# study-game-engines/directx-renderer-kurth

Measured on AMD Instinct MI355X. Metric: physics steps/sec at 100k rigid bodies, higher is better.
Workload: dtype f32; 1 GPU; c3: 100k mixed colliders (sphere/capsule/OBB), dt 1/120 s, 30 solver iterations; bodies=100000, broadphase_pairs=611032, manifolds=251275, contacts=317267, joints=0, recoveries=0, parallelism=1 gpu

## Files before the change

### directx-renderer-kurth_amd/csrc/k_broad.hip

```cpp
#include "world.h"
#include <rocprim/rocprim.hpp>

#define CELL_BIAS (1 << 20)
#define CELL_MASK ((1u << 21) - 1u)
#define EMPTY_CELL 0xFFFFFFFFu

MI_DEV u64 packCell(i32 ix, i32 iy, i32 iz) { return ((u64)(u32)(ix & CELL_MASK)) | ((u64)(u32)(iy & CELL_MASK) << 21) | ((u64)(u32)(iz & CELL_MASK) << 42); }
MI_DEV u32 hashCell(u64 k, u32 mask)
{
	k ^= k >> 30; k *= 0xbf58476d1ce4e5b9ull; k ^= k >> 27; k *= 0x94d049bb133111ebull; k ^= k >> 31;
	return (u32)k & mask;
}
MI_DEV i32 cellCoord(float v, float invCell)
{
	float c = floorf(v * invCell);
	c = fminf(fmaxf(c, -(float)(CELL_BIAS - 2)), (float)(CELL_BIAS - 2));
	return (i32)c + CELL_BIAS;
}
MI_DEV u32 cellTag(i32 ix, i32 iy, i32 iz) { return ((u32)ix & 0x3FFu) | (((u32)iy & 0x3FFu) << 10) | (((u32)iz & 0x3FFu) << 20); }
MI_DEV bool aabbOverlap(float4 amin, float4 amax, float4 bmin, float4 bmax)
{
	if (amax.x < bmin.x || amin.x > bmax.x) return false;
	if (amax.y < bmin.y || amin.y > bmax.y) return false;
	if (amax.z < bmin.z || amin.z > bmax.z) return false;
	return true;
}

__global__ void __launch_bounds__(256) k_cell_assign(const u32* __restrict__ activeCols, u32 hashMask, const float4* __restrict__ aabbMin, const float4* __restrict__ aabbMax,
	u32* __restrict__ counters, u32* __restrict__ hashKey, u32* __restrict__ cellCount)
{
	const u32 gid = blockIdx.x * blockDim.x + threadIdx.x;
	if (gid == 0) { counters[CTR_FIRST_LARGE] = 0xFFFFFFFFu; counters[CTR_FIRST_INACTIVE] = 0xFFFFFFFFu; counters[CTR_PAIR_OVERFLOW] = 0u; }
	const u32 n = counters[CTR_ACTIVE_COLS];
	float maxExtent = fmaxf(__uint_as_float(counters[CTR_CELL_SIZE]), 1e-3f);
	float cell = maxExtent * 1.001f;
	float invCell = 1.f / cell;
	for (u32 a = gid; a < n; a += gridDim.x * blockDim.x)
	{
		const u32 i = activeCols[a];
		float4 mn = aabbMin[i], mx = aabbMax[i];
		float e = fmaxf(fmaxf(mx.x - mn.x, mx.y - mn.y), mx.z - mn.z);
		u32 h;
		if (mn.x > mx.x) { h = hashMask + 2; }
		else if (e > maxExtent) { h = hashMask + 1; }
		else { h = hashCell(packCell(cellCoord(mn.x, invCell), cellCoord(mn.y, invCell), cellCoord(mn.z, invCell)), hashMask); }
		hashKey[i] = h;
		atomicAdd(&cellCount[h], 1u);
	}
}

__global__ void __launch_bounds__(256) k_cell_place(const u32* __restrict__ counters, const u32* __restrict__ activeCols, const u32* __restrict__ hashKey, u32* __restrict__ cellBase, u32* __restrict__ tmpIdx)
{
	const u32 n = counters[CTR_ACTIVE_COLS];
	for (u32 a = blockIdx.x * blockDim.x + threadIdx.x; a < n; a += gridDim.x * blockDim.x) { const u32 i = activeCols[a]; tmpIdx[atomicAdd(&cellBase[hashKey[i]], 1u)] = i; }
}
__global__ void __launch_bounds__(256) k_cell_rank(u32* __restrict__ counters, u32 hashMask, const u32* __restrict__ hashKey, const u32* __restrict__ cellBase, const u32* __restrict__ cellCount, const u32* __restrict__ tmpIdx,
	const float4* __restrict__ aabbMin, const float4* __restrict__ aabbMax, float4* __restrict__ sBox, u32* __restrict__ cellRange)
{
	const u32 n = counters[CTR_ACTIVE_COLS];
	const float cell = fmaxf(__uint_as_float(counters[CTR_CELL_SIZE]), 1e-3f) * 1.001f;
	const float invCell = 1.f / cell;
	if (blockIdx.x == 0 && threadIdx.x == 0) counters[CTR_CELL_SIZE_USED] = counters[CTR_CELL_SIZE];
	for (u32 t = blockIdx.x * blockDim.x + threadIdx.x; t < n; t += gridDim.x * blockDim.x)
	{
		const u32 i = tmpIdx[t], h = hashKey[i], end = cellBase[h], start = end - cellCount[h];
		u32 rank = t - start;
		if (h != hashMask + 2u) { rank = 0; for (u32 u = start; u < end; ++u) rank += tmpIdx[u] < i ? 1u : 0u; }
		const u32 pos = start + rank;
		float4 mn = aabbMin[i], mx = aabbMax[i];
		mx.w = __uint_as_float(cellTag(cellCoord(mn.x, invCell), cellCoord(mn.y, invCell), cellCoord(mn.z, invCell)));
		mn.w = __uint_as_float(i);
		sBox[2 * pos] = mn; sBox[2 * pos + 1] = mx;
		if (t == start)
		{
			if (h <= hashMask) { cellRange[2 * h] = start; cellRange[2 * h + 1] = end; }
			else counters[h == hashMask + 1 ? CTR_FIRST_LARGE : CTR_FIRST_INACTIVE] = start;
		}
	}
}

#define PAIR_SLAB 32
#define PAIR_LANES 16
#define PAIR_NO_TAG 0xFFFFFFFFu
enum { MODE_SLAB = 0, MODE_WRITE = 1 };
MI_DEV uint2 pairRange(const uint4* ranges, u32 r) { return make_uint2(ranges[r].x, ranges[r].y); }
MI_DEV const float4* pairBox(const float4* __restrict__ sBox, u32 u) { return (const float4*)((const char*)sBox + u * 32u); }
template <int MODE>
__global__ void __launch_bounds__(256) k_pairs(u32 nc, u32 hashMask, const float4* __restrict__ sBox, const uint2* __restrict__ cellRange, u32* __restrict__ counters,
	u32* __restrict__ pairCount, const u32* __restrict__ pairOffset, uint2* __restrict__ out, u32 pairCap)
{
	__shared__ uint4 sRange[256 / PAIR_LANES][PAIR_LANES];
	u32 gid = blockIdx.x * blockDim.x + threadIdx.x;
	u32 t = gid / PAIR_LANES, g = gid % PAIR_LANES;
	const uint4* __restrict__ ranges = sRange[threadIdx.x / PAIR_LANES];
	bool valid = t < nc;
	u32 nEnd = min(counters[CTR_FIRST_INACTIVE], min(nc, counters[CTR_ACTIVE_COLS]));
	u32 firstLarge = min(counters[CTR_FIRST_LARGE], nEnd);
	bool live = valid && t < nEnd;
	if (MODE == MODE_WRITE) live = live && pairCount[t] > PAIR_SLAB;
	float4 amin = make_float4(0.f, 0.f, 0.f, 0.f), amax = amin;
	u32 me = 0;
	u32 s = 0, len = 0, ntag = PAIR_NO_TAG;
	if (live)
	{
		amin = sBox[2 * t]; amax = sBox[2 * t + 1];
		me = __float_as_uint(amin.w);
		if (t >= firstLarge) { if (g == 0) { s = firstLarge; len = t - firstLarge; } }
		else if (g == 14) { s = firstLarge; len = nEnd - firstLarge; }
		else if (g < 14)
		{
			const float invCell = 1.f / (fmaxf(__uint_as_float(counters[CTR_CELL_SIZE_USED]), 1e-3f) * 1.001f);
			i32 ix = cellCoord(amin.x, invCell), iy = cellCoord(amin.y, invCell), iz = cellCoord(amin.z, invCell);
			i32 o = 13 + (i32)g;
			i32 dz = o / 9 - 1, dy = (o / 3) % 3 - 1, dx = o % 3 - 1;
			bool reach = true;
			if (dx > 0 && cellCoord(amax.x, invCell) == ix) reach = false;
			if (dy > 0 && cellCoord(amax.y, invCell) == iy) reach = false;
			if (dz > 0 && cellCoord(amax.z, invCell) == iz) reach = false;
			if (reach)
			{
				ntag = cellTag(ix + dx, iy + dy, iz + dz);
				u32 h = hashCell(packCell(ix + dx, iy + dy, iz + dz), hashMask);
				uint2 range = cellRange[h];
				if (range.x != EMPTY_CELL) { s = range.x; const u32 e = g == 0 ? min(range.y, t) : range.y; len = e > s ? e - s : 0u; }
			}
		}
	}
	u32 end = len;
	for (u32 d = 1; d < PAIR_LANES; d <<= 1) { u32 v = __shfl_up(end, d, PAIR_LANES); if (g >= d) end += v; }
	sRange[threadIdx.x / PAIR_LANES][g] = make_uint4(end, s - (end - len), ntag, 0u);
	__syncthreads();
	const u32 T = ranges[PAIR_LANES - 1].x;
	const u32 chunk = (T + PAIR_LANES - 1u) / PAIR_LANES;
	const u32 lo = min(g * chunk, T), hi = min(lo + chunk, T);
	u32 r0 = 0;
#pragma unroll
	for (u32 k = 0; k < PAIR_LANES - 1u; ++k) r0 += ranges[k].x <= lo ? 1u : 0u;
	u32 n = 0;
	u32 hit0 = 0, hit1 = 0, hit2 = 0, hit3 = 0;
	if (lo < hi)
	{
		u32 r = r0; uint2 cur = pairRange(ranges, r);
		for (u32 p = lo; p < hi; p += 4u)
		{
			float4 bmin[4], bmax[4]; u32 from = 0;
#pragma unroll
			for (u32 k = 0; k < 4u; ++k) if (p + k < hi)
			{
				while (p + k >= cur.x) cur = pairRange(ranges, ++r);
				const float4* box = pairBox(sBox, cur.y + p + k);
				from |= r << (4u * k); bmin[k] = box[0]; bmax[k] = box[1];
			}
#pragma unroll
			for (u32 k = 0; k < 4u; ++k)
			{
				if (p + k >= hi) continue;
				const u32 want = ranges[(from >> (4u * k)) & 15u].z;
				if (want != PAIR_NO_TAG && __float_as_uint(bmax[k].w) != want) continue;
				if (aabbOverlap(amin, amax, bmin[k], bmax[k]))
				{
					u32 partner = __float_as_uint(bmin[k].w);
					if (n == 0) hit0 = partner; else if (n == 1) hit1 = partner; else if (n == 2) hit2 = partner; else if (n == 3) hit3 = partner;
					++n;
				}
			}
		}
	}
	u32 incl = n;
	for (u32 d = 1; d < PAIR_LANES; d <<= 1) { u32 v = __shfl_up(incl, d, PAIR_LANES); if (g >= d) incl += v; }
	u32 total = __shfl(incl, PAIR_LANES - 1, PAIR_LANES);
	u32 pos = incl - n;
	if (MODE == MODE_SLAB && valid && g == 0) { pairCount[t] = live ? total : 0; if (total > PAIR_SLAB) counters[CTR_PAIR_OVERFLOW] = 1; }
	if (!n) return;
	size_t base = (MODE == MODE_WRITE) ? (size_t)pairOffset[t] : (size_t)t * PAIR_SLAB;
	u32 room = (MODE == MODE_WRITE) ? 0xFFFFFFFFu : PAIR_SLAB;
	if (n <= 4)
	{
		for (u32 k = 0; k < n; ++k)
		{
			u32 partner = k == 0 ? hit0 : (k == 1 ? hit1 : (k == 2 ? hit2 : hit3));
			if (pos + k < room && (MODE == MODE_SLAB || base + pos + k < pairCap)) out[base + pos + k] = make_uint2(me, partner);
		}
		return;
	}
	u32 r = r0; uint2 cur = pairRange(ranges, r);
	for (u32 p = lo; p < hi; ++p)
	{
		while (p >= cur.x) cur = pairRange(ranges, ++r);
		const float4* box = pairBox(sBox, cur.y + p);
		float4 bmin = box[0], bmax = box[1];
		const u32 want = ranges[r].z;
		if (want != PAIR_NO_TAG && __float_as_uint(bmax.w) != want) continue;
		if (!aabbOverlap(amin, amax, bmin, bmax)) continue;
		if (pos < room && (MODE == MODE_SLAB || base + pos < pairCap)) out[base + pos] = make_uint2(me, __float_as_uint(bmin.w));
		++pos;
	}
}

__global__ void __launch_bounds__(256) k_pairs_pack(u32 nc, const u32* __restrict__ pairCount, const u32* __restrict__ pairOffset, const uint2* __restrict__ slab,
	uint2* __restrict__ pairs, u32 pairCap)
{
	u32 i = blockIdx.x * blockDim.x + threadIdx.x;
	u32 t = i / PAIR_SLAB, k = i % PAIR_SLAB;
	if (t >= nc || k >= pairCount[t]) return;
	u32 dst = pairOffset[t] + k;
	if (dst < pairCap) pairs[dst] = slab[i];
}

__global__ void k_finish_pair_count(u32 launched, const u32* __restrict__ pairCount, const u32* __restrict__ pairOffset, u32* __restrict__ counters, const double* __restrict__ sapPartial, u32 sapBlocks, u32 stepParity)
{
	double acc[7] = { 0., 0., 0., 0., 0., 0., 0. };
	for (u32 b = threadIdx.x; b < sapBlocks; b += 64u) for (int k = 0; k < 7; ++k) acc[k] += sapPartial[(size_t)b * 7 + k];
	for (int o = 32; o > 0; o >>= 1) for (int k = 0; k < 7; ++k) acc[k] += __shfl_xor(acc[k], o);
	if (threadIdx.x == 0 && blockIdx.x == 0)
	{
		const u32 na = counters[CTR_ACTIVE_COLS], nc = min(na, launched);
		counters[CTR_ACTIVE_OVERFLOW] = na > launched ? 1u : 0u;
		counters[CTR_NUM_PAIRS] = nc ? pairOffset[nc - 1] + pairCount[nc - 1] : 0;
		counters[CTR_CELL_SIZE] = 0;
		const double n = acc[6] > 0. ? acc[6] : 1.;
		const double vx = acc[3] - acc[0] * acc[0] / n, vy = acc[4] - acc[1] * acc[1] / n, vz = acc[5] - acc[2] * acc[2] / n;
		counters[CTR_SAP_AXIS + (stepParity ^ 1u)] = (vx > vy) ? ((vx > vz) ? 0u : 2u) : ((vy > vz) ? 1u : 2u);
	}
}

static void ensureTemp(World& w, size_t bytes)
{
	if (bytes > w.tempStorage.cap) w.tempStorage.ensure(bytes + bytes / 2 + 4096, w.stream);
}
void prim_sort_pairs_u32(World& w, const u32* kin, u32* kout, const u32* vin, u32* vout, u32 n, u32 bits)
{
	if (!n) return;
	size_t bytes = 0;
	MI_CHECK(rocprim::radix_sort_pairs(nullptr, bytes, kin, kout, vin, vout, n, 0, bits, w.stream));
	ensureTemp(w, bytes);
	MI_CHECK(rocprim::radix_sort_pairs(w.tempStorage.p, bytes, kin, kout, vin, vout, n, 0, bits, w.stream));
}
void prim_sort_pairs_u32_u64(World& w, const u32* kin, u32* kout, const u64* vin, u64* vout, u32 n, u32 bits)
{
	if (!n) return;
	size_t bytes = 0;
	MI_CHECK(rocprim::radix_sort_pairs(nullptr, bytes, kin, kout, vin, vout, n, 0, bits, w.stream));
	ensureTemp(w, bytes);
	MI_CHECK(rocprim::radix_sort_pairs(w.tempStorage.p, bytes, kin, kout, vin, vout, n, 0, bits, w.stream));
}
void prim_exclusive_scan_u32(World& w, const u32* in, u32* out, u32 n)
{
	if (!n) return;
	size_t bytes = 0;
	MI_CHECK(rocprim::exclusive_scan(nullptr, bytes, in, out, 0u, n, rocprim::plus<u32>(), w.stream));
	ensureTemp(w, bytes);
	MI_CHECK(rocprim::exclusive_scan(w.tempStorage.p, bytes, in, out, 0u, n, rocprim::plus<u32>(), w.stream));
}

static u32 log2ceil(u32 v) { u32 b = 0; while ((1u << b) < v) ++b; return b; }

void launch_broadphase_count(World& w)
{
	if (!w.nc) return;
	const u32 bound = (u32)std::min<u64>(w.nc, (u64)w.estActiveCols + w.estActiveCols / 8u + 2048u);
	w.pairBound = bound;
	dim3 grid(std::max(1u, (bound + 255u) / 256u)), block(256);
	u32 H = w.hashTableSize, mask = H - 1;
	hipLaunchKernelGGL(k_cell_assign, grid, block, 0, w.stream, w.actCols.p, mask, w.aabbMin.p, w.aabbMax.p, w.dCounters.p, w.hashKey.p, w.cellCount.p);
	prim_exclusive_scan_u32(w, w.cellCount.p, w.cellBase.p, H + 3);
	hipLaunchKernelGGL(k_cell_place, grid, block, 0, w.stream, w.dCounters.p, w.actCols.p, w.hashKey.p, w.cellBase.p, w.sortIdx.p);
	hipLaunchKernelGGL(k_cell_rank, grid, block, 0, w.stream, w.dCounters.p, mask, w.hashKey.p, w.cellBase.p, w.cellCount.p, w.sortIdx.p, w.aabbMin.p, w.aabbMax.p, w.sBox.p, w.cellStart.p);
	w.pairSlab.ensure((size_t)bound * PAIR_SLAB, w.stream);
	if (w.lastError) return;
	hipLaunchKernelGGL(HIP_KERNEL_NAME(k_pairs<MODE_SLAB>), dim3((u32)(((size_t)bound * PAIR_LANES + 255) / 256)), block, 0, w.stream, bound, mask, w.sBox.p, (const uint2*)w.cellStart.p, w.dCounters.p,
		w.pairCount.p, w.pairOffset.p, w.pairSlab.p, 0u);
	prim_exclusive_scan_u32(w, w.pairCount.p, w.pairOffset.p, bound);
	hipLaunchKernelGGL(k_finish_pair_count, dim3(1), dim3(64), 0, w.stream, bound, w.pairCount.p, w.pairOffset.p, w.dCounters.p, w.sapPartial.p, w.sapBlocks, w.stats.numInternalSteps & 1u);
}

void launch_broadphase_write(World& w, u32 numPairs, bool slabOverflow)
{
	const u32 nc = w.pairBound;
	if (!nc || !numPairs) return;
	hipLaunchKernelGGL(k_pairs_pack, dim3((u32)(((size_t)nc * PAIR_SLAB + 255) / 256)), dim3(256), 0, w.stream, nc, w.pairCount.p, w.pairOffset.p, w.pairSlab.p, w.pairs.p, (u32)w.pairCap);
	if (slabOverflow)
		hipLaunchKernelGGL(HIP_KERNEL_NAME(k_pairs<MODE_WRITE>), dim3((u32)(((size_t)nc * PAIR_LANES + 255) / 256)), dim3(256), 0, w.stream, nc, w.hashTableSize - 1, w.sBox.p, (const uint2*)w.cellStart.p, w.dCounters.p, w.pairCount.p, w.pairOffset.p, w.pairs.p, (u32)w.pairCap);
}
```

### directx-renderer-kurth_amd/csrc/world.h

```cpp
#pragma once
#include "mi_common.h"
#include "../../include/mi_physics.h"
#include <vector>
#include <string>
#include <algorithm>

struct mi_distance_constraint { float localAnchorA[3], localAnchorB[3], globalLength; };
struct mi_ball_constraint { float localAnchorA[3], localAnchorB[3]; };
struct mi_fixed_constraint { float initialInvRotationDifference[4], localAnchorA[3], localAnchorB[3]; };
struct mi_hinge_constraint
{
	float localAnchorA[3], localAnchorB[3], localHingeAxisA[3], localHingeAxisB[3];
	float minRotationLimit, maxRotationLimit, maxMotorTorque; u32 motorType; float motorVelocity;
	float localHingeTangentA[3], localHingeBitangentA[3], localHingeTangentB[3];
};
struct mi_cone_twist_constraint
{
	float localAnchorA[3], localAnchorB[3], localLimitAxisA[3], localLimitAxisB[3];
	float localLimitTangentA[3], localLimitBitangentA[3], localLimitTangentB[3];
	float swingLimit, twistLimit; u32 swingMotorType; float swingMotorVelocity, maxSwingMotorTorque, swingMotorAxis;
	u32 twistMotorType; float twistMotorVelocity, maxTwistMotorTorque;
};
struct mi_slider_constraint
{
// ... 8 lines not shown
static const u32 MI_JOINT_UPDATE_FLOATS[MI_JOINT_TYPES] = { 20, 20, 36, 56, 80, 72 };

template <typename T> struct DevBuf
{
	T* p = nullptr; size_t cap = 0;
	void ensure(size_t n, hipStream_t s, bool keep = false);
	void release();
};

struct JointSet
{
	std::vector<uint8_t> pods;
	std::vector<u32> a, b;
	std::vector<uint8_t> alive;
	DevBuf<uint8_t> dPods; DevBuf<uint2> dPairs; DevBuf<float> dUpdate;
	std::vector<u32> order;
	std::vector<u32> colorStart;
	u32 count() const { return (u32)a.size(); }
	u32 numColors() const { return colorStart.empty() ? 0u : (u32)colorStart.size() - 1u; }
};

enum
{
	CTR_NUM_PAIRS = 0,
	CTR_NUM_VALID = 1,
	CTR_NUM_MANIFOLDS = 2,
	CTR_EPA_COUNT = 3,
	CTR_NUM_COLORS = 4,
	CTR_FIRST_LARGE = 5,
	CTR_LAST_ROUND = 6,
	CTR_OVERFLOW = 7,
	CTR_CELL_SIZE = 8,
	CTR_NUM_ACTIVE = 9,
	CTR_NUM_CONTACTS = 10,
	CTR_PAIR_OVERFLOW = 11,
	CTR_FIRST_INACTIVE = 12,
	CTR_FLOW_STATUS = 13,
	CTR_FLOW_PROBES = 14,
	CTR_EPA_COUNT_HULL = 15,
	CTR_BUCKET_START = 16,
	CTR_KEY_START = 96,
	CTR_COLOR_BARRIER = 360,
	CTR_SAP_AXIS = 368,
	CTR_CL_SCRATCH = 371,
	CTR_CL_LEFT = 372,
	CTR_ACTIVE_BODIES = 377,
	CTR_ACTIVE_COLS = 378,
	CTR_ACTIVE_OVERFLOW = 379,
	CTR_CELL_SIZE_USED = 380,
	CTR_EVENT_COUNT = 416,
	CTR_EVENT_OVERFLOW = 417,
	CTR_TERRAIN_BASE = 418,
	CTR_TERRAIN_OVERFLOW = 419,
	CTR_CL_NUM_TASKS = 424,
	CTR_CL_STATUS = 429,
	CTR_CL_SHARED = 430,
	CTR_CL_PHASE_COUNT = 431,
	CTR_CL_BBOX = 436,
	CTR_CL_REMAIN = 442,
	CTR_VALIDATE = 448,
	CTR_NARROW_LIMITS = 450,
	CTR_WORDS = 512,
};
struct CtrRange { u32 first, words; };
static constexpr CtrRange CTR_LAYOUT[] =
{
	{ CTR_NUM_PAIRS, 1 }, { CTR_NUM_VALID, 1 }, { CTR_NUM_MANIFOLDS, 1 }, { CTR_EPA_COUNT, 1 }, { CTR_NUM_COLORS, 1 }, { CTR_FIRST_LARGE, 1 }, { CTR_LAST_ROUND, 1 }, { CTR_OVERFLOW, 1 },
	{ CTR_CELL_SIZE, 1 }, { CTR_NUM_ACTIVE, 1 }, { CTR_NUM_CONTACTS, 1 }, { CTR_PAIR_OVERFLOW, 1 }, { CTR_FIRST_INACTIVE, 1 }, { CTR_FLOW_STATUS, 1 }, { CTR_FLOW_PROBES, 1 }, { CTR_EPA_COUNT_HULL, 1 },
	{ CTR_BUCKET_START, 65 }, { CTR_KEY_START, (MI_MAX_COLORS + 1) * 4 + 1 }, { CTR_COLOR_BARRIER, 4 }, { CTR_SAP_AXIS, 2 }, { CTR_CL_SCRATCH, 1 }, { CTR_CL_LEFT, 5 },
	{ CTR_ACTIVE_BODIES, 1 }, { CTR_ACTIVE_COLS, 1 }, { CTR_ACTIVE_OVERFLOW, 1 }, { CTR_CELL_SIZE_USED, 1 }, { CTR_EVENT_COUNT, 1 }, { CTR_EVENT_OVERFLOW, 1 }, { CTR_TERRAIN_BASE, 1 }, { CTR_TERRAIN_OVERFLOW, 1 },
	{ CTR_CL_NUM_TASKS, 5 }, { CTR_CL_STATUS, 1 }, { CTR_CL_SHARED, 1 }, { CTR_CL_PHASE_COUNT, 5 }, { CTR_CL_BBOX, 6 }, { CTR_CL_REMAIN, 6 }, { CTR_VALIDATE, 2 }, { CTR_NARROW_LIMITS, 5 },
};
constexpr bool ctrLayoutDisjoint() { u32 end = 0; for (const CtrRange& r : CTR_LAYOUT) { if (r.first < end) return false; end = r.first + r.words; } return end <= CTR_WORDS; }
static_assert(ctrLayoutDisjoint(), "CTR_*: an entry reaches into the next one (or past CTR_WORDS), or CTR_LAYOUT is not in ascending order");
#define MI_REPLAY_WIDTH 8u
#define CL_MAX_PARTS 4u
#define CL_CURVE_PARTS 2u
#define CL_MAX_PHASES (CL_MAX_PARTS + 1u)
#define CL_MAX_TASKS 512u
#define CL_BODY_STRIDE 4096u
#define CL_MAX_JOINT_CLASSES 64u
#define CL_TASK_MAX_JOINTS 512u
#define MI_NUM_SCHEDULE_KEYS ((MI_MAX_COLORS + 1) * 4)

struct StepRecord
{
	u32 numPairs = 0, truePairs = 0;
	bool slabOverflow = false;
	u32 axis = 0;
	float dt = 0.f; u32 iters = 0;
	bool cluster = false;
	bool unsettled = false;
	u32 jointPath = MI_JOINT_PATH_NONE;
	bool counted = true;
};

struct World
{
	int device = 0;
	hipStream_t stream = nullptr;
	int lastError = 0; std::string lastErrorText;

	struct HBody { float pos[3], rot[4]; float localCOG[3], invMass, invInertia[9]; float gravityFactor, linDamp, angDamp; float v[3], w[3], force[3], torque[3]; std::vector<u32> colliders; bool removed = false; };
	struct HCollider { float shape[10]; float restitution, friction, density; u32 type, body; float spos[3], srot[4]; u32 zoneType, zoneIndex; };
	struct HField { float force[3]; float pos[3], rot[4]; u32 hasTransform, numColliders; };
	struct HTrigger { float pos[3], rot[4]; u32 numColliders; };
	std::vector<HField> fields; std::vector<HTrigger> triggers;
	u32 terrainChunksPerDim = 0, terrainSlotsPerCollider = 8, terrainMinSlots = 8192; float terrainChunkSize = 0.f, terrainAmplitude = 1.f, terrainMinCorner[3] = { 0.f, 0.f, 0.f }, terrainMaterial[3] = { 0.f, 0.f, 0.f };
	std::vector<uint16_t> hTerrainHeights; std::vector<u32> hTerrainValid;
	DevBuf<uint16_t> terrainHeights; DevBuf<u32> terrainValid, terrainCounts, terrainOffsets;
	u32 terrainSlotCap() const { return terrainChunksPerDim ? std::max(terrainMinSlots, terrainSlotsPerCollider * (u32)colliders.size()) : 0u; }
	hipEvent_t countersEvent = nullptr;
	struct HClothConstraint { u32 a, b; float restDistance, inverseMassSum; u32 color; };
	struct HCloth
	{
		float width, height, totalMass, stiffness, damping, gravityFactor, oldTotalMass, oldStiffness; u32 gridX, gridY;
		std::vector<float> pos, prev, vel, invMass;
		std::vector<HClothConstraint> constraints;
	};
	std::vector<HCloth> cloths;
	bool clothsDirty = true, clothStateOnDevice = false;
	u32 clothIterations[3] = { 0, 1, 0 };
	DevBuf<float> clothPlanes; u32 clothStride = 0;
	DevBuf<uint2> clothAB; DevBuf<float2> clothRestIms; DevBuf<float4> clothTemp; DevBuf<uint8_t> clothDescs; DevBuf<u32> clothList;
	u32 numSmallCloths = 0, maxSmallClothParticles = 0;
	void uploadCloths(); void downloadCloths();
	bool fieldsDirty = true;
	bool collisionBeginEvents = false, collisionEndEvents = false;
	std::vector<HBody> bodies;
	std::vector<HCollider> colliders;
	struct HHull { std::vector<float> vertices; std::vector<u32> triangles; float aabbMin[3], aabbMax[3]; };
	std::vector<HHull> hulls;
	JointSet joints[MI_JOINT_TYPES];
	u32 numJointKernels() const { u32 n = 0; for (const JointSet& js : joints) n += js.numColors(); return n; }
	u32 numSortedJoints() const { u32 n = 0; for (const JointSet& js : joints) n += (u32)js.order.size(); return n; }
	bool topologyDirty = true;
	bool jointsDirty = true;
	bool stateOnDevice = false;

	u32 nb = 0, nc = 0;
	DevBuf<float4> pose, pose0, poseLerp, vel, bprops, force, cog, invIw;
	DevBuf<ColliderRec> colLocal, colWorld;
	DevBuf<float4> colStaticPose, aabbMin, aabbMax;
	DevBuf<float4> hullVerts, hullInfo;
	DevBuf<uint8_t> aliveMask;
	DevBuf<uint8_t> simMask;
	DevBuf<uint8_t> slabCode; DevBuf<u32> slabFresh; u32 slabRank = 0, slabSize = 0, slabAxis = 0, slabStamp = 0; float slabLo = 0.f, slabHi = 0.f, slabMargin = 0.f;
	DevBuf<u32> cellCount, cellBase;
	DevBuf<u32> hashKey, sortIdx, cellStart , largeFlag, largeScan, largeList, pairCount, pairOffset;
	DevBuf<float4> sBox;
	DevBuf<u32> actBodies, actCols, actBlockCount, actBlockBase, colBody; bool activeDirty = true; u32 estActiveBodies = 0, estActiveCols = 0, pairBound = 0, sapBlocks = 0;
	DevBuf<double> sapPartial;
	DevBuf<uint2> pairs, pairSlab;
	u32 hashTableSize = 0;
	DevBuf<u32> pairKey, pairKeySorted; DevBuf<uint2> pairsSorted;
	DevBuf<ManifoldRec> manifolds;
	DevBuf<u64> bodyMask, claim; DevBuf<u32> mColor, mKey, mKeySorted, mIdx, mOrder;
	DevBuf<uint4> actIds;
	DevBuf<u32> epaList; DevBuf<float4> gjkSimplex;
	DevBuf<float4> rowPlanes, rowShared; DevBuf<float2> rowLambda; DevBuf<uint4> rowIds;
	DevBuf<u64> flow;
	bool validate = false;
	bool replayReferenceOrder = false; DevBuf<u32> replayEntries; std::vector<u32> replayHost; u32 replayBatches = 0;
	u32 scheduleReferenceBatches(const std::vector<uint4>& ids, u32 numPositions);
	bool useCluster = true;
	u32 clusterBlocksLimit = 0, clusterFailStreak = 0, clusterTaskWeight = 64u * 1000u, clusterTaskWeightLater = 64u * 500u;
	bool clusterSortDue = true; u32 clusterSortAge = 0, clusterSortBodies = 0;
	u32 clusterLdsBytes = 0, clusterBlocks = 0, clusterCooldown = 0;
	DevBuf<u32> clKeys, clKeysSorted, clVals, clSorted, clRank, clWsum, clCum, clPhaseMask, clTaskKey, clTaskPos, clPre, clLocal, clEntry, clTaskCount, clTaskStart, clBodyList, clSharedSlot;
	DevBuf<uint8_t> clTasks;
	DevBuf<float4> clRowScratch;
	DevBuf<u32> clJointBodyMask; bool clJointListsValid = false;
	DevBuf<u32> clCompLabel, clLeftList;
	bool compIdle = false;
	DevBuf<u32> clChunk; u32 clChunkJointVersion = ~0u; bool clChunkWithJoints = false;
	DevBuf<u32> clRep, clJointTask, clJointPos, clJointCount, clJointStart, clJointList; DevBuf<uint4> clJointTable; DevBuf<uint2> clTaskJoints; DevBuf<u32> clJointClassStart;
	bool useClusterJoints = true;
	u32 clNumJoints = 0, clNumJointClasses = 0; bool clJointsInCluster = false;
	DevBuf<u64> flowTrace;
	u32 flowEpoch = 0;
	DevBuf<float4> velBackup; u32 flowTestAbortStep = ~0u;
	void recoverFlow(); int resolvePendingFlow();
	DevBuf<float4> fieldForce;
	DevBuf<u32> fieldMask; u32 fieldWords = 0;
	float globalForce[3] = { 0.f, 0.f, 0.f }; bool anyGlobalForce = false;
	DevBuf<u64> triggerSet[2], collisionSet[2]; u32 triggerSetSize = 0, collisionSetSize = 0, triggerCur = 0, collisionCur = 0;
	DevBuf<uint8_t> eventRing; u32 eventCap = 1u << 16;
	std::vector<u64> restoredTriggerKeys, restoredCollisionKeys;
	std::vector<mi_event> pendingEvents;
	void uploadFields(); void ensureEventBuffers(u32 numPairs);
	DevBuf<uint8_t> tempStorage;
	DevBuf<u32> sortHist;
	DevBuf<u32> dCounters; u32* hCounters = nullptr;
	size_t pairCap = 0, rowCap = 0;

	u32 iterations = 30;
	u32 coloringRounds = 24;
	DevBuf<u64> colorHash[2]; u32 colorHashCur = 0, colorHashSize = 0, stepsSinceFullColoring = 0;
	bool forceFullColoring = true;
	u32 lastNumManifolds = 0;
	mi_stats stats = {};
	StepRecord last;
	static const u32 STAGE_RING = 32;
	std::vector<hipEvent_t> stageEvents;
	u32 ringHead = 0, ringPending = 0, accTimed = 0; double accMs[5] = { 0, 0, 0, 0, 0 };
	bool timeStages = false;
	void harvestTiming();
	double sumContacts = 0, sumManifolds = 0, sumColors = 0, sumPairs = 0, sumProbes = 0; u32 sumSteps = 0;
	void countPreviousStep(); void refreshCounters();
	u32 jointVersion = 0;
	bool jointPodsOnDevice = false;
	u32 jointGeneration = 0;
	void pullJointPods();
	void jointsChanged();
	DevBuf<u32> bodyColStart, bodyColList; DevBuf<uint4> hullTris; DevBuf<uint2> hullTriRange; bool interactTablesValid = false;
	void buildInteractTables();
	DevBuf<float4> rcHostRays, rcHostHits;
	DevBuf<float4> rcLeafBox, rcNodes; DevBuf<u32> rcCount, rcKeys, rcKeysSorted, rcVals, rcValsSorted, rcParentInt, rcParentLeaf;
	DevBuf<u32> rcTerrainTiles, rcTerrainChunkRange; bool rcTerrainTableValid = false;

	World(int dev);
	~World();
	void fail(int code, const std::string& what);
	void upload();
	void uploadJoints();
	void downloadState();
	int stepInternal(float dt, u32 iterations);
	int step(float* timer, const mi_physics_settings* s, float dt);
};

extern thread_local World* g_currentWorld;
static inline u32 nextPow2(u32 v) { u32 p = 1; while (p < v) p <<= 1; return p; }
void recalculateProperties(World& w, World::HBody& rb);
void ensurePairBuffers(World& w, size_t numPairs);

void launch_active_lists(World& w);
void launch_restore_velocities(World& w);
u32 active_grid(u32 estimate, u32 total);
void launch_build_colliders(World& w);
void launch_broadphase_count(World& w);
void launch_broadphase_write(World& w, u32 numPairs, bool slabOverflow);
void launch_narrowphase(World& w, u32 numPairs, u32 stepParity);
void launch_zone_overlap(World& w, u32 numPairs);
void launch_integrate_forces(World& w, float dt, bool backupVelocities);
void launch_heightmap(World& w, u32 numPairs, u32 slotCap);
void launch_cloth(World& w, float dt);
u32 cloth_lds_particle_limit();
void launch_apply_fields(World& w);
void launch_trigger_events(World& w);
void launch_collision_events(World& w, u32 numPairs);
void launch_coloring(World& w, u32 numPairs);
void launch_contact_init(World& w, u32 numPairs, float dt);
void launch_solve_replay(World& w, u32 numBatches);
void launch_solve_contacts_iteration(World& w, const u32* gridBlocks, u32 numColors, u32 firstTail, bool serialBucket);
bool cluster_available(World& w);
void launch_active_list(World& w, u32 numPairs);
void launch_cluster_build(World& w, u32 numPairs);
void launch_cluster_solve(World& w, u32 itBegin, u32 itEnd);
bool cluster_solves_joints(const World& w);
void launch_integrate_velocities(World& w, float dt);
void launch_joint_init(World& w, float dt);
void launch_joint_solve_iteration(World& w);
void launch_and_mask(World& w);
void launch_slab_classify(World& w);
void launch_slab_pack(World& w, void* left, void* right, u32 capacity);
void launch_slab_unpack(World& w, const void* left, const void* right, u32 capacity);
void launch_validate(World& w, u32 stage, u32 numPairs);
void launch_copy_pose0(World& w);
void launch_interaction_batch(World& w, u32 numRays, u32 firstBody, u32 bodiesPerRay, const float* dRays, int32_t* dOutBody);
void launch_raycast(World& w, u32 numRays, const float* dRays, u32 flags, mi_ray_hit* dOutHits);
void launch_raycast_terrain(World& w, u32 numRays, const float* dRays, u32 flags, mi_ray_hit* dOutHits);
void launch_lerp_pose(World& w, float t);
void csort_pairs_u32(World& w, const u32* keys, u32* keysOut, const u32* vals, u32* valsOut, u32 n, u32 numBuckets);
void csort_pairs_u64(World& w, const u32* keys, u32* keysOut, const u64* vals, u64* valsOut, u32 n, u32 numBuckets);
```

### directx-renderer-kurth_amd/csrc/world.hip

```cpp
#include "world.h"
#include <cstdio>
#include <cstring>
#include <atomic>

thread_local std::string g_createError;
thread_local World* g_currentWorld = nullptr;

void mi_set_error(hipError_t e, const char* file, int line)
{
	char buf[512];
	snprintf(buf, sizeof(buf), "HIP error %d (%s) at %s:%d", (int)e, hipGetErrorString(e), file, line);
	if (g_currentWorld) { if (!g_currentWorld->lastError) { g_currentWorld->lastError = MI_ERR_HIP; g_currentWorld->lastErrorText = buf; } }
	else g_createError = buf;
}

template <typename T> void DevBuf<T>::ensure(size_t n, hipStream_t s, bool keep)
{
	if (n <= cap) return;
	size_t newCap = std::max(n, cap + cap / 2);
	T* np = nullptr;
	MI_CHECK(hipMalloc((void**)&np, newCap * sizeof(T)));
	if (!np) return;
	if (keep && p && cap) { MI_CHECK(hipMemcpyAsync(np, p, cap * sizeof(T), hipMemcpyDeviceToDevice, s)); MI_CHECK(hipStreamSynchronize(s)); }
	if (p) MI_CHECK(hipFree(p));
	p = np; cap = newCap;
}
template <typename T> void DevBuf<T>::release() { if (p) { (void)hipFree(p); p = nullptr; cap = 0; } }

template struct DevBuf<float4>; template struct DevBuf<float2>; template struct DevBuf<uint2>; template struct DevBuf<uint4>; template struct DevBuf<u32>;
template struct DevBuf<double>; template struct DevBuf<u64>; template struct DevBuf<uint8_t>; template struct DevBuf<uint16_t>; template struct DevBuf<float>; template struct DevBuf<ColliderRec>; template struct DevBuf<ManifoldRec>;

World::World(int dev) : device(dev)
{
	g_currentWorld = this;
	MI_CHECK(hipSetDevice(dev));
	MI_CHECK(hipStreamCreateWithFlags(&stream, hipStreamNonBlocking));
	MI_CHECK(hipHostMalloc((void**)&hCounters, CTR_WORDS * sizeof(u32), hipHostMallocDefault));
	if (hCounters) memset(hCounters, 0, CTR_WORDS * sizeof(u32));
	dCounters.ensure(CTR_WORDS, stream);
	if (dCounters.p) MI_CHECK(hipMemsetAsync(dCounters.p, 0, CTR_WORDS * sizeof(u32), stream));
	stageEvents.resize(STAGE_RING * 6);
	for (auto& e : stageEvents) MI_CHECK(hipEventCreateWithFlags(&e, hipEventDisableSystemFence));
	MI_CHECK(hipEventCreateWithFlags(&countersEvent, hipEventDisableTiming));
	validate = getenv("MI_PHYSICS_VALIDATE") != nullptr;
	useCluster = getenv("MI_PHYSICS_NO_CLUSTER") == nullptr;
	useClusterJoints = getenv("MI_CLUSTER_NO_JOINTS") == nullptr;
	if (const char* e = getenv("MI_FLOW_TEST_ABORT")) flowTestAbortStep = (u32)atoi(e);
	if (const char* e = getenv("MI_CLUSTER_TASK")) { clusterTaskWeight = 64u * (u32)std::max(16, atoi(e)); clusterTaskWeightLater = std::min(clusterTaskWeight, clusterTaskWeightLater); }
	if (getenv("MI_PHYSICS_REPLAY")) replayReferenceOrder = true;
	if (const char* e = getenv("MI_CLUSTER_BLOCKS")) clusterBlocksLimit = (u32)std::max(1, atoi(e));
	if (const char* e = getenv("MI_CLUSTER_TASK_LATER")) clusterTaskWeightLater = 64u * (u32)std::max(16, atoi(e));
	if (dCounters.p)
	{
		u32 box[6] = { 0xFFFFFFFFu, 0xFFFFFFFFu, 0xFFFFFFFFu, 0u, 0u, 0u };
		MI_CHECK(hipMemcpyAsync(dCounters.p + CTR_CL_BBOX, box, sizeof(box), hipMemcpyHostToDevice, stream));
		MI_CHECK(hipStreamSynchronize(stream));
	}
}

World::~World()
{
	g_currentWorld = this;
	if (stream) (void)hipStreamSynchronize(stream);
	DevBuf<float4>* f4[] = { &pose, &pose0, &poseLerp, &vel, &bprops, &force, &cog, &invIw, &colStaticPose, &aabbMin, &aabbMax, &sBox, &rowPlanes, &rowShared };
	for (auto b : f4) b->release();
	DevBuf<u32>* u4[] = { &hashKey, &sortIdx, &cellStart, &largeFlag, &largeScan, &largeList, &pairCount, &pairOffset, &pairKey, &pairKeySorted,
		&mColor, &mKey, &mKeySorted, &mIdx, &mOrder, &dCounters };
	for (auto b : u4) b->release();
	colLocal.release(); colWorld.release(); pairs.release(); pairsSorted.release(); manifolds.release(); bodyMask.release(); claim.release();
	rowLambda.release(); rowIds.release(); tempStorage.release(); actIds.release(); epaList.release(); gjkSimplex.release(); pairSlab.release(); simMask.release();
	for (auto& js : joints) { js.dPods.release(); js.dPairs.release(); js.dUpdate.release(); }
	bodyColStart.release(); bodyColList.release(); hullTris.release(); hullTriRange.release();
	rcHostRays.release(); rcHostHits.release(); rcLeafBox.release(); rcNodes.release(); rcCount.release(); rcKeys.release(); rcKeysSorted.release(); rcVals.release(); rcValsSorted.release(); rcParentInt.release(); rcParentLeaf.release(); rcTerrainTiles.release(); rcTerrainChunkRange.release();
	for (auto& e : stageEvents) if (e) (void)hipEventDestroy(e);
	if (countersEvent) (void)hipEventDestroy(countersEvent);
	if (hCounters) (void)hipHostFree(hCounters);
	if (stream) (void)hipStreamDestroy(stream);
	g_currentWorld = nullptr;
}

void World::fail(int code, const std::string& what) { if (!lastError) { lastError = code; lastErrorText = what; } }

struct MassProps { M3 inertia; V3 cog; float mass; };

static M3 mzero() { M3 r; memset(&r, 0, sizeof(r)); return r; }
static M3 mscaleH(const M3& a, float s) { M3 r; const float* p = &a.m00; float* q = &r.m00; for (int i = 0; i < 9; ++i) q[i] = p[i] * s; return r; }
static M3 msub(const M3& a, const M3& b) { M3 r; const float* p = &a.m00; const float* q = &b.m00; float* o = &r.m00; for (int i = 0; i < 9; ++i) o[i] = p[i] - q[i]; return r; }
static M3 mouter(V3 a, V3 b)
{
	V3 c0 = a * b.x, c1 = a * b.y, c2 = a * b.z;
	M3 r; r.m00 = c0.x; r.m10 = c0.y; r.m20 = c0.z; r.m01 = c1.x; r.m11 = c1.y; r.m21 = c1.z; r.m02 = c2.x; r.m12 = c2.y; r.m22 = c2.z;
	return r;
}
static M3 minvert(const M3& m)
{
	M3 inv;
	inv.m00 = m.m11 * m.m22 - m.m21 * m.m12; inv.m01 = m.m02 * m.m21 - m.m22 * m.m01; inv.m02 = m.m01 * m.m12 - m.m11 * m.m02;
	inv.m10 = m.m12 * m.m20 - m.m22 * m.m10; inv.m11 = m.m00 * m.m22 - m.m20 * m.m02; inv.m12 = m.m02 * m.m10 - m.m12 * m.m00;
	inv.m20 = m.m10 * m.m21 - m.m20 * m.m11; inv.m21 = m.m01 * m.m20 - m.m21 * m.m00; inv.m22 = m.m00 * m.m11 - m.m10 * m.m01;
	float det = m.m00 * (m.m11 * m.m22 - m.m21 * m.m12) - m.m01 * (m.m10 * m.m22 - m.m20 * m.m12) + m.m02 * (m.m10 * m.m21 - m.m20 * m.m11);
	if (det == 0.f) return mzero();
	return mscaleH(inv, 1.f / det);
}

static MassProps colliderMassProps(const World::HCollider& c, const World& w)
{
	MassProps r; r.inertia = mzero(); r.cog = v3s(0.f); r.mass = 0.f;
	const float* s = c.shape;
	switch (c.type)
	{
		case MI_HULL:
		{
			Q4 rot = q4(s[0], s[1], s[2], s[3]); V3 pos = v3(s[4], s[5], s[6]);
			const World::HHull& g = w.hulls[(u32)s[7]];
			const float s60 = 1.f / 60.f, s120 = 1.f / 120.f;
			M3 C; C.m00 = s60; C.m01 = s120; C.m02 = s120; C.m10 = s120; C.m11 = s60; C.m12 = s120; C.m20 = s120; C.m21 = s120; C.m22 = s60;
			float totalMass = 0.f; M3 totalCov = mzero(); V3 totalCOG = v3s(0.f);
			for (size_t f = 0; f + 2 < g.triangles.size(); f += 3)
			{
				const float* pa = &g.vertices[3 * g.triangles[f]]; const float* pb = &g.vertices[3 * g.triangles[f + 1]]; const float* pc = &g.vertices[3 * g.triangles[f + 2]];
				V3 w1 = pos + rot * v3(pa[0], pa[1], pa[2]), w2 = pos + rot * v3(pb[0], pb[1], pb[2]), w3 = pos + rot * v3(pc[0], pc[1], pc[2]);
				M3 A; A.m00 = w1.x; A.m01 = w2.x; A.m02 = w3.x; A.m10 = w1.y; A.m11 = w2.y; A.m12 = w3.y; A.m20 = w1.z; A.m21 = w2.z; A.m22 = w3.z;
				float detA = A.m00 * (A.m11 * A.m22 - A.m21 * A.m12) - A.m01 * (A.m10 * A.m22 - A.m20 * A.m12) + A.m02 * (A.m10 * A.m21 - A.m20 * A.m11);
				M3 cov = (mscaleH(A, detA) * C) * mtranspose(A);
				float volume = 1.f / 6.f * detA;
				V3 cg = (w1 + w2 + w3) * 0.25f;
				totalMass += volume;
				totalCov = madd(totalCov, cov);
				totalCOG += cg * volume;
			}
			totalCOG = totalCOG / totalMass;
			M3 Cp = msub(totalCov, mscaleH(mouter(totalCOG, totalCOG), totalMass));
			r.cog = totalCOG;
			r.mass = totalMass * c.density;
			r.inertia = mscaleH(msub(mscaleH(midentity(), Cp.m00 + Cp.m11 + Cp.m22), Cp), c.density);
		} break;
		case MI_SPHERE:
		{
			float radius = s[3];
			float sqRadiusPI = MI_PI * (radius * radius);
			r.mass = (4.f / 3.f * sqRadiusPI * radius) * c.density;
			r.cog = v3(s[0], s[1], s[2]);
			r.inertia = mscaleH(midentity(), 2.f / 5.f * r.mass * radius * radius);
		} break;
		case MI_CAPSULE:
		{
			V3 pA = v3(s[0], s[1], s[2]), pB = v3(s[3], s[4], s[5]); float radius = s[6];
			V3 axis = pA - pB;
			if (axis.y < 0.f) axis *= -1.f;
			float height = length(axis);
			axis *= (1.f / height);
			M3 rot = quaternionToMat3(rotateFromTo(v3(0.f, 1.f, 0.f), axis));
			float sqRadius = radius * radius;
			float sqRadiusPI = MI_PI * sqRadius;
			float volume = 4.f / 3.f * sqRadiusPI * radius + sqRadiusPI * length(pA - pB);
			r.mass = volume * c.density;
			r.cog = (pA + pB) * 0.5f;
			float cylinderMass = c.density * sqRadiusPI * height;
			float hemiSphereMass = c.density * 2.f / 3.f * sqRadiusPI * radius;
			float sqCapsuleHeight = height * height;
			M3 I = mzero();
			I.m11 = sqRadius * cylinderMass * 0.5f;
			I.m00 = I.m22 = I.m11 * 0.5f + cylinderMass * sqCapsuleHeight / 12.f;
			float temp0 = hemiSphereMass * 2.f * sqRadius / 5.f;
			I.m11 += temp0 * 2.f;
			float temp1 = height * 0.5f;
			float temp2 = temp0 + hemiSphereMass * (temp1 * temp1 + 3.f / 8.f * sqCapsuleHeight);
			I.m00 += temp2 * 2.f;
			I.m22 += temp2 * 2.f;
			r.inertia = mtranspose(rot) * I * rot;
		} break;
		case MI_CYLINDER:
		{
			V3 pA = v3(s[0], s[1], s[2]), pB = v3(s[3], s[4], s[5]); float radius = s[6];
			V3 axis = pA - pB;
			if (axis.y < 0.f) axis *= -1.f;
			float height = length(axis);
			axis *= (1.f / height);
			M3 rot = quaternionToMat3(rotateFromTo(v3(0.f, 1.f, 0.f), axis));
			float sqRadiusPI = MI_PI * radius * radius;
			r.mass = (sqRadiusPI * length(pA - pB)) * c.density;
			r.cog = (pA + pB) * 0.5f;
			float sqRadius = radius * radius;
			float sqHeight = height * height;
			M3 I = mzero();
			I.m11 = sqRadius * r.mass * 0.5f;
			I.m00 = I.m22 = 1.f / 12.f * r.mass * (3.f * sqRadius + sqHeight);
			r.inertia = mtranspose(rot) * I * rot;
		} break;
		case MI_AABB:
		{
			V3 lo = v3(s[0], s[1], s[2]), hi = v3(s[3], s[4], s[5]);
			V3 d0 = hi - lo;
			r.mass = (d0.x * d0.y * d0.z) * c.density;
			r.cog = (lo + hi) * 0.5f;
			V3 d = ((hi - lo) * 0.5f) * 2.f;
			r.inertia.m00 = 1.f / 12.f * r.mass * (d.y * d.y + d.z * d.z);
			r.inertia.m11 = 1.f / 12.f * r.mass * (d.x * d.x + d.z * d.z);
			r.inertia.m22 = 1.f / 12.f * r.mass * (d.x * d.x + d.y * d.y);
		} break;
		case MI_OBB:
		{
			Q4 q = q4(s[0], s[1], s[2], s[3]); V3 radius = v3(s[7], s[8], s[9]);
// ... 251 lines not shown
```

Measured before the change: 544.0 steps/s.

## Fuse slab pack and overflow pair rewrite into one persistent finish kernel

Replaces the separate slab-pack kernel and the conditional full-grid MODE_WRITE pair kernel with a single persistent-block kernel. Each block walks segments of colliders, copies slab pairs with vectorized 16-byte loads, and queues overflowing colliders in LDS so the per-cell pair search reruns only for them. This removes one launch and the full-size overflow grid, at the cost of extra block barriers, a static device-property query, and a grid capped at a few blocks per CU. An env var can limit the block count.

```diff
diff --git a/directx-renderer-kurth_amd/csrc/k_broad.hip b/directx-renderer-kurth_amd/csrc/k_broad.hip
--- a/directx-renderer-kurth_amd/csrc/k_broad.hip
+++ b/directx-renderer-kurth_amd/csrc/k_broad.hip
@@ -86,18 +86,10 @@
 MI_DEV uint2 pairRange(const uint4* ranges, u32 r) { return make_uint2(ranges[r].x, ranges[r].y); }
 MI_DEV const float4* pairBox(const float4* __restrict__ sBox, u32 u) { return (const float4*)((const char*)sBox + u * 32u); }
 template <int MODE>
-__global__ void __launch_bounds__(256) k_pairs(u32 nc, u32 hashMask, const float4* __restrict__ sBox, const uint2* __restrict__ cellRange, u32* __restrict__ counters,
-	u32* __restrict__ pairCount, const u32* __restrict__ pairOffset, uint2* __restrict__ out, u32 pairCap)
-{
-	__shared__ uint4 sRange[256 / PAIR_LANES][PAIR_LANES];
-	u32 gid = blockIdx.x * blockDim.x + threadIdx.x;
-	u32 t = gid / PAIR_LANES, g = gid % PAIR_LANES;
+MI_DEV void pairVisit(u32 t, u32 g, bool valid, bool live, u32 nEnd, u32 firstLarge, u32 hashMask, const float4* __restrict__ sBox, const uint2* __restrict__ cellRange, u32* __restrict__ counters,
+	u32* __restrict__ pairCount, const u32* __restrict__ pairOffset, uint2* __restrict__ out, u32 pairCap, uint4 (*sRange)[PAIR_LANES])
+{
 	const uint4* __restrict__ ranges = sRange[threadIdx.x / PAIR_LANES];
-	bool valid = t < nc;
-	u32 nEnd = min(counters[CTR_FIRST_INACTIVE], min(nc, counters[CTR_ACTIVE_COLS]));
-	u32 firstLarge = min(counters[CTR_FIRST_LARGE], nEnd);
-	bool live = valid && t < nEnd;
-	if (MODE == MODE_WRITE) live = live && pairCount[t] > PAIR_SLAB;
 	float4 amin = make_float4(0.f, 0.f, 0.f, 0.f), amax = amin;
 	u32 me = 0;
 	u32 s = 0, len = 0, ntag = PAIR_NO_TAG;
@@ -197,14 +189,78 @@
 	}
 }
 
-__global__ void __launch_bounds__(256) k_pairs_pack(u32 nc, const u32* __restrict__ pairCount, const u32* __restrict__ pairOffset, const uint2* __restrict__ slab,
-	uint2* __restrict__ pairs, u32 pairCap)
-{
-	u32 i = blockIdx.x * blockDim.x + threadIdx.x;
-	u32 t = i / PAIR_SLAB, k = i % PAIR_SLAB;
-	if (t >= nc || k >= pairCount[t]) return;
-	u32 dst = pairOffset[t] + k;
-	if (dst < pairCap) pairs[dst] = slab[i];
+__global__ void __launch_bounds__(256) k_pairs(u32 nc, u32 hashMask, const float4* __restrict__ sBox, const uint2* __restrict__ cellRange, u32* __restrict__ counters,
+	u32* __restrict__ pairCount, const u32* __restrict__ pairOffset, uint2* __restrict__ out, u32 pairCap)
+{
+	__shared__ uint4 sRange[256 / PAIR_LANES][PAIR_LANES];
+	u32 gid = blockIdx.x * blockDim.x + threadIdx.x;
+	u32 t = gid / PAIR_LANES, g = gid % PAIR_LANES;
+	bool valid = t < nc;
+	u32 nEnd = min(counters[CTR_FIRST_INACTIVE], min(nc, counters[CTR_ACTIVE_COLS]));
+	u32 firstLarge = min(counters[CTR_FIRST_LARGE], nEnd);
+	pairVisit<MODE_SLAB>(t, g, valid, valid && t < nEnd, nEnd, firstLarge, hashMask, sBox, cellRange, counters, pairCount, pairOffset, out, pairCap, sRange);
+}
+
+#define FINISH_SEG 1024u
+__global__ void __launch_bounds__(256) k_pairs_finish(u32 nc, u32 hashMask, const float4* __restrict__ sBox, const uint2* __restrict__ cellRange, u32* __restrict__ counters,
+	u32* __restrict__ pairCount, const u32* __restrict__ pairOffset, const uint2* __restrict__ slab, uint2* __restrict__ pairs, u32 pairCap, u32 serveOverflow)
+{
+	__shared__ uint4 sRange[256 / PAIR_LANES][PAIR_LANES];
+	__shared__ u32 sQueue[FINISH_SEG];
+	__shared__ u32 sQueueLen;
+	const u32 per = (nc + gridDim.x - 1u) / gridDim.x;
+	const u32 first = min(blockIdx.x * per, nc), last = min(first + per, nc);
+	const u32 lane = threadIdx.x & 63u, wave = threadIdx.x >> 6;
+	const u32 nEnd = min(counters[CTR_FIRST_INACTIVE], min(nc, counters[CTR_ACTIVE_COLS]));
+	const u32 firstLarge = min(counters[CTR_FIRST_LARGE], nEnd);
+	for (u32 seg = first; seg < last; seg += FINISH_SEG)
+	{
+		const u32 segEnd = min(seg + FINISH_SEG, last);
+		if (threadIdx.x == 0) sQueueLen = 0u;
+		__syncthreads();
+		for (u32 t0 = seg + wave * 16u; t0 < segEnd; t0 += 64u)
+		{
+			const u32 tl = t0 + (lane & 15u);
+			u32 cnt = 0, off = 0;
+			if (lane < 16u && tl < segEnd) { cnt = pairCount[tl]; off = pairOffset[tl]; }
+			const bool over = serveOverflow && cnt > PAIR_SLAB;
+			const u64 mask = __ballot(over);
+			if (mask)
+			{
+				u32 at = 0;
+				if (lane == 0u) at = atomicAdd(&sQueueLen, (u32)__popcll(mask));
+				at = __shfl(at, 0);
+				if (over) sQueue[at + (u32)__popcll(mask & ((1ull << lane) - 1ull))] = tl;
+			}
+			const u32 c = lane >> 2, k0 = (lane & 3u) * 8u, t = t0 + c;
+			const u32 n = min(__shfl(cnt, (int)c), (u32)PAIR_SLAB), dst = __shfl(off, (int)c);
+			if (k0 < n)
+			{
+				const uint4* __restrict__ src = (const uint4*)(slab + (size_t)t * PAIR_SLAB + k0);
+				uint4 v[4];
+#pragma unroll
+				for (u32 j = 0; j < 4u; ++j) if (k0 + 2u * j < n) v[j] = src[j];
+#pragma unroll
+				for (u32 j = 0; j < 4u; ++j)
+				{
+					const u32 k = k0 + 2u * j;
+					if (k < n && dst + k < pairCap) pairs[dst + k] = make_uint2(v[j].x, v[j].y);
+					if (k + 1u < n && dst + k + 1u < pairCap) pairs[dst + k + 1u] = make_uint2(v[j].z, v[j].w);
+				}
+			}
+		}
+		__syncthreads();
+		const u32 queued = sQueueLen;
+		for (u32 i = 0; i < queued; i += 256u / PAIR_LANES)
+		{
+			const u32 qi = i + threadIdx.x / PAIR_LANES;
+			const bool live = qi < queued;
+			const u32 t = live ? sQueue[qi] : 0u;
+			__syncthreads();
+			pairVisit<MODE_WRITE>(t, threadIdx.x % PAIR_LANES, live, live && t < nEnd, nEnd, firstLarge, hashMask, sBox, cellRange, counters, pairCount, pairOffset, pairs, pairCap, sRange);
+		}
+		__syncthreads();
+	}
 }
 
 __global__ void k_finish_pair_count(u32 launched, const u32* __restrict__ pairCount, const u32* __restrict__ pairOffset, u32* __restrict__ counters, const double* __restrict__ sapPartial, u32 sapBlocks, u32 stepParity)
@@ -268,7 +324,7 @@
 	hipLaunchKernelGGL(k_cell_rank, grid, block, 0, w.stream, w.dCounters.p, mask, w.hashKey.p, w.cellBase.p, w.cellCount.p, w.sortIdx.p, w.aabbMin.p, w.aabbMax.p, w.sBox.p, w.cellStart.p);
 	w.pairSlab.ensure((size_t)bound * PAIR_SLAB, w.stream);
 	if (w.lastError) return;
-	hipLaunchKernelGGL(HIP_KERNEL_NAME(k_pairs<MODE_SLAB>), dim3((u32)(((size_t)bound * PAIR_LANES + 255) / 256)), block, 0, w.stream, bound, mask, w.sBox.p, (const uint2*)w.cellStart.p, w.dCounters.p,
+	hipLaunchKernelGGL(k_pairs, dim3((u32)(((size_t)bound * PAIR_LANES + 255) / 256)), block, 0, w.stream, bound, mask, w.sBox.p, (const uint2*)w.cellStart.p, w.dCounters.p,
 		w.pairCount.p, w.pairOffset.p, w.pairSlab.p, 0u);
 	prim_exclusive_scan_u32(w, w.pairCount.p, w.pairOffset.p, bound);
 	hipLaunchKernelGGL(k_finish_pair_count, dim3(1), dim3(64), 0, w.stream, bound, w.pairCount.p, w.pairOffset.p, w.dCounters.p, w.sapPartial.p, w.sapBlocks, w.stats.numInternalSteps & 1u);
@@ -278,7 +334,10 @@
 {
 	const u32 nc = w.pairBound;
 	if (!nc || !numPairs) return;
-	hipLaunchKernelGGL(k_pairs_pack, dim3((u32)(((size_t)nc * PAIR_SLAB + 255) / 256)), dim3(256), 0, w.stream, nc, w.pairCount.p, w.pairOffset.p, w.pairSlab.p, w.pairs.p, (u32)w.pairCap);
-	if (slabOverflow)
-		hipLaunchKernelGGL(HIP_KERNEL_NAME(k_pairs<MODE_WRITE>), dim3((u32)(((size_t)nc * PAIR_LANES + 255) / 256)), dim3(256), 0, w.stream, nc, w.hashTableSize - 1, w.sBox.p, (const uint2*)w.cellStart.p, w.dCounters.p, w.pairCount.p, w.pairOffset.p, w.pairs.p, (u32)w.pairCap);
-}
+	static int numCUs = 0;
+	if (!numCUs) { hipDeviceProp_t prop; MI_CHECK(hipGetDeviceProperties(&prop, w.device)); numCUs = prop.multiProcessorCount > 0 ? prop.multiProcessorCount : 256; }
+	u32 blocks = std::min<u32>(4u * (u32)numCUs, (nc + 63u) / 64u);
+	if (w.collisionBlocksLimit) blocks = std::min(blocks, w.collisionBlocksLimit);
+	hipLaunchKernelGGL(k_pairs_finish, dim3(blocks), dim3(256), 0, w.stream, nc, w.hashTableSize - 1, w.sBox.p, (const uint2*)w.cellStart.p, w.dCounters.p, w.pairCount.p, w.pairOffset.p,
+		(const uint2*)w.pairSlab.p, w.pairs.p, (u32)w.pairCap, slabOverflow ? 1u : 0u);
+}
diff --git a/directx-renderer-kurth_amd/csrc/world.h b/directx-renderer-kurth_amd/csrc/world.h
--- a/directx-renderer-kurth_amd/csrc/world.h
+++ b/directx-renderer-kurth_amd/csrc/world.h
@@ -184,6 +184,7 @@
 	DevBuf<u32> actBodies, actCols, actBlockCount, actBlockBase, colBody; bool activeDirty = true; u32 estActiveBodies = 0, estActiveCols = 0, pairBound = 0, sapBlocks = 0;
 	DevBuf<double> sapPartial;
 	DevBuf<uint2> pairs, pairSlab;
+	u32 collisionBlocksLimit = 0;
 	u32 hashTableSize = 0;
 	DevBuf<u32> pairKey, pairKeySorted; DevBuf<uint2> pairsSorted;
 	DevBuf<ManifoldRec> manifolds;
diff --git a/directx-renderer-kurth_amd/csrc/world.hip b/directx-renderer-kurth_amd/csrc/world.hip
--- a/directx-renderer-kurth_amd/csrc/world.hip
+++ b/directx-renderer-kurth_amd/csrc/world.hip
@@ -49,6 +49,7 @@
 	if (const char* e = getenv("MI_CLUSTER_TASK")) { clusterTaskWeight = 64u * (u32)std::max(16, atoi(e)); clusterTaskWeightLater = std::min(clusterTaskWeight, clusterTaskWeightLater); }
 	if (getenv("MI_PHYSICS_REPLAY")) replayReferenceOrder = true;
 	if (const char* e = getenv("MI_CLUSTER_BLOCKS")) clusterBlocksLimit = (u32)std::max(1, atoi(e));
+	if (const char* e = getenv("MI_COLLISION_BLOCKS")) collisionBlocksLimit = (u32)std::max(1, atoi(e));
 	if (const char* e = getenv("MI_CLUSTER_TASK_LATER")) clusterTaskWeightLater = 64u * (u32)std::max(16, atoi(e));
 	if (dCounters.p)
 	{
```

After: 546.2 steps/s, median of 6. No clear change (+0.4%).
